# facebookresearch/vggsfm

Measured on AMD Instinct MI355X. Metric: BA LM-iterations/sec, higher is better.
Workload: dtype f64

## Files before the change

### vggsfm_amd/csrc/ba.hip

```cpp
#include <type_traits>

#include "camera_model.hpp"
#include "../../include/vggsfm_amd.h"

namespace vgg {

int cholesky_solve_enqueue(double* A, double* b, int n, double* inv_blocks, int32_t* device_fail, const int32_t* skip_flag,
                           hipStream_t st, const CholOverlap* overlap, int split_a, int split_b, const int32_t* first_blk,
                           bool flags_cleared);
int32_t* cholesky_dataflow_flags(double* ws, int n, size_t* count);
size_t cholesky_workspace_bytes(int n);
void dataflow_signal(int32_t* flag, hipStream_t st);

constexpr int kGroup = 16;
#ifndef VGG_OFFDIAG_OCC
#define VGG_OFFDIAG_OCC 3
#endif
#ifndef VGG_DIAG_OCC
#define VGG_DIAG_OCC 4
#endif
#ifndef VGG_DIAG_FULL_DEPTH
#define VGG_DIAG_FULL_DEPTH 2
#endif
#ifndef VGG_OFF_FULL_DEPTH
// ... 17 lines not shown
#ifndef VGG_CP_OCC_RHS
#define VGG_CP_OCC_RHS 2
#endif
#ifndef VGG_CP_OCC
#define VGG_CP_OCC 2
#endif
#ifndef VGG_ABLATE
#define VGG_ABLATE 0
#endif
constexpr int kSub = 32;
constexpr int kMaxWG = 2048;
constexpr int kCamSplitMax = 16;
constexpr int kCamNV = 48;
constexpr int kPackPad = 1024;

struct Ctl {
  double radius, decrease_factor, x_cost, initial_cost, gmax_cams, gmax, cand_cost, mcc, step_norm, rel;
  int32_t iteration, done, termination, need_lin, scale_ready, invalid_streak, num_succ, num_unsucc;
  int32_t linear_fail, accept, rank, world, grad_logged, pad0, pad1, pad2;
};

struct Dims {
  int C, P, O, NI, model, kd, only_k, shared, BDp, n_red, kdsh, loss;
  double loss_scale;
};

constexpr int kYc = 12;
static inline size_t y_slot_doubles(const Dims& d) { return (d.shared || d.kd == 0) ? (size_t)kYc : (size_t)d.BDp * 3; }

struct Ws {
  Ctl* ctl;
  vgg_ba_iteration* log;
  double *cand_q, *cand_t, *cand_intr, *cand_pts;
  double *scale_c, *scale_p, *colsq_c, *dsq_c, *dy;
  uint8_t* active;
  double* lin;
  double *U, *g, *costc;
  double* sys;
  double *S, *rhs;
  double* S2;
  double* gmax_pts;
  double* stepsum;
  double *G, *hs, *Ms;
  double *pdamp;
  double* T;
  double* part_B;
  double* part_F;
  double* packed;
  size_t packed_count;
  double* pk_mine;
  double* pk_gathered;
  double* cam_part;
  double* cam_split;
  double* Y;
  size_t y_bytes;
  double* chol_inv;
  double* tile_part;
  int32_t* batch_flags;
  double *Zp, *rz_part, *part_Q;
  unsigned long long* split_off;
  double* rz;
  int tile_rhs;
  double* lin_cand;
  double *U_cand, *g_cand, *cost_cand;
  size_t lin_count, sys_count, total_bytes;
};

static inline size_t align_up(size_t x, size_t a) { return (x + a - 1) / a * a; }


static Dims make_dims(const vgg_ba_problem* pb) {
  Dims d;
  d.C = pb->num_cams; d.P = pb->num_pts; d.O = pb->num_obs; d.NI = pb->num_intr; d.model = pb->camera_model;
  const int rf = pb->refine_focal ? 1 : 0, rk = (pb->refine_extra && pb->camera_model == kSimpleRadial) ? 1 : 0;
  d.kd = rf + rk;
  d.only_k = (!rf && rk) ? 1 : 0;
  d.shared = (pb->num_intr == 1) ? 1 : 0;
  d.BDp = 6 + d.kd;
  d.n_red = 6 * d.C + d.kd * d.NI;
  d.kdsh = d.shared ? d.kd : 0;
  d.loss = pb->loss; d.loss_scale = pb->loss_scale;
  return d;
}

struct Tuning { int lpp, longt, cam_wgs, point_wgs, tile_rhs; };
static Tuning g_tuning = {0, -1, 0, 0, 2};

static Ws carve(const Dims& d, int max_iters, int num_chunks, int num_segments, void* base) {
  Ws w;
  size_t off = 0;
  auto take = [&](size_t bytes) { size_t o = off; off = align_up(off + bytes, 256); return (char*)base + o; };
  w.ctl = (Ctl*)take(sizeof(Ctl));
  w.log = (vgg_ba_iteration*)take(sizeof(vgg_ba_iteration) * (size_t)(max_iters + 2));
  w.cand_q = (double*)take(8ull * 4 * d.C); w.cand_t = (double*)take(8ull * 3 * d.C);
  w.cand_intr = (double*)take(8ull * 4 * d.NI); w.cand_pts = (double*)take(8ull * 3 * d.P);
  w.scale_c = (double*)take(8ull * d.n_red); w.scale_p = (double*)take(8ull * 3 * d.P);
  w.colsq_c = (double*)take(8ull * d.n_red); w.dsq_c = (double*)take(8ull * d.n_red);
  w.dy = (double*)take(8ull * d.n_red);
  w.active = (uint8_t*)take(d.n_red);
  w.lin_count = (size_t)d.C * d.BDp * d.BDp + (size_t)d.C * d.BDp + d.C;
  w.lin = (double*)take(8ull * w.lin_count);
  w.U = w.lin; w.g = w.U + (size_t)d.C * d.BDp * d.BDp; w.costc = w.g + (size_t)d.C * d.BDp;
  w.sys_count = (size_t)d.n_red * d.n_red + d.n_red;
  w.sys = (double*)take(8ull * w.sys_count);
  w.S = w.sys; w.rhs = w.S + (size_t)d.n_red * d.n_red;
  w.S2 = (double*)take(8ull * (size_t)d.n_red * d.n_red);
  w.packed_count = (size_t)d.n_red * (d.n_red + 1) / 2 + d.n_red;
  w.packed = (double*)take(8ull * (w.packed_count + 2 * kPackPad));
  w.pk_mine = (double*)take(8ull * (w.packed_count + 2));
  w.pk_gathered = (double*)take(8ull * (w.packed_count + 3 * kPackPad));
  w.gmax_pts = (double*)take(64);
  w.stepsum = (double*)take(64);
  w.G = (double*)take(8ull * 6 * d.P); w.hs = (double*)take(8ull * 3 * d.P);
  w.pdamp = (double*)take(8ull * 3 * d.P);
  w.Ms = (double*)take(8ull * 3 * (d.kdsh ? d.kdsh : 1) * d.P);
  w.T = (double*)take(8ull * d.C * d.BDp * (1 + d.kdsh));
  w.part_B = (double*)take(8ull * kMaxWG);
  w.part_F = (double*)take(8ull * kMaxWG * 4);
  w.cam_part = (double*)take(8ull * (d.C + 1) * 3);
  w.cam_split = (double*)take(8ull * (size_t)d.C * kCamSplitMax * kCamNV);
  w.y_bytes = 8ull * ((size_t)(num_segments > 0 ? num_segments : 0) + 1) * kGroup * y_slot_doubles(d);
  w.Y = (double*)take(w.y_bytes);
  w.chol_inv = (double*)take(cholesky_workspace_bytes(d.n_red));
  {
    const size_t bdt = d.shared ? 6 : d.BDp;
    w.tile_part = (double*)take(8ull * (size_t)(num_chunks > 0 ? num_chunks : 1) * bdt * bdt * 256);
  }
  w.batch_flags = (int32_t*)take(64);
  w.Zp = (double*)take(8ull * 9 * (d.P > 0 ? d.P : 1));
  w.rz_part = (double*)take(8ull * (size_t)(num_chunks > 0 ? num_chunks : 1) * kGroup * 6 * 3);
  w.part_Q = (double*)take(8ull * kMaxWG * 8);
  w.rz = (double*)take(8ull * (size_t)((d.C + kGroup - 1) / kGroup) * kGroup * 6 * 3);
  w.split_off = (unsigned long long*)take(8ull * 2 * ((size_t)d.n_red + 2));
  w.lin_cand = (double*)take(8ull * w.lin_count);
  w.U_cand = w.lin_cand; w.g_cand = w.U_cand + (size_t)d.C * d.BDp * d.BDp; w.cost_cand = w.g_cand + (size_t)d.C * d.BDp;
  w.tile_rhs = 0;
  w.total_bytes = off;
  return w;
}

struct DevProblem {
  Dims d;
  const double *cam_q, *cam_t, *intr, *pts;
  const int32_t *row_ptr, *obs_cam, *col_ptr, *cobs_pt, *obs_slot;
  const float2 *obs_uv, *cobs_uv;
  const uint8_t *cam_const, *intr_const, *pt_const;
};

static DevProblem dev_problem(const vgg_ba_problem* pb, const Dims& d) {
  DevProblem p;
  p.d = d; p.cam_q = pb->cam_q; p.cam_t = pb->cam_t; p.intr = pb->intr; p.pts = pb->pts;
  p.row_ptr = pb->row_ptr; p.obs_cam = pb->obs_cam; p.col_ptr = pb->col_ptr; p.cobs_pt = pb->cobs_pt;
  p.obs_slot = pb->obs_slot;
  p.obs_uv = (const float2*)pb->obs_uv; p.cobs_uv = (const float2*)pb->cobs_uv;
  p.cam_const = pb->cam_const; p.intr_const = pb->intr_const; p.pt_const = pb->pt_const;
  return p;
}

template <int N>
struct ObsPf {
  static_assert(N == 2 || N == 4, "prefetch depth");
  int c0 = 0, c1 = 0, c2 = 0, c3 = 0, s0 = 0, s1 = 0, s2 = 0, s3 = 0;
  float2 u0 = make_float2(0.f, 0.f), u1 = make_float2(0.f, 0.f), u2 = make_float2(0.f, 0.f), u3 = make_float2(0.f, 0.f);
  template <bool SLOT>
  __device__ __forceinline__ void load(const int32_t* cam, const float2* uv, const int32_t* slot, int o0, int o1, int stride, int sl) {
    int o = o0 + sl;
    if (o < o1) { c0 = cam[o]; u0 = uv[o]; if (SLOT) s0 = slot[o]; }
    o += stride;
// ... 82 lines not shown
    const double s = wave_sum(v[i]);
    if (lane == 0) lds[wave * NV + i] = s;
  }
  __syncthreads();
  if (threadIdx.x < NV) out[threadIdx.x] = lds[threadIdx.x] + lds[NV + threadIdx.x] + lds[2 * NV + threadIdx.x] + lds[3 * NV + threadIdx.x];
  __syncthreads();
}

__global__ void init_kernel(DevProblem pb, Ws w, vgg_ba_options opt, int rank, int world) {
  const Dims& d = pb.d;
  const int j = blockIdx.x * blockDim.x + threadIdx.x;
  if (j == 0) {
    Ctl c;
    memset(&c, 0, sizeof(c));
    c.radius = opt.initial_trust_region_radius; c.decrease_factor = 2.0; c.need_lin = 1; c.rank = rank; c.world = world;
    *w.ctl = c;
    w.gmax_pts[0] = 0; for (int i = 0; i < 4; ++i) w.stepsum[i] = 0;
  }
  if (j < d.n_red) {
    bool act;
    if (j < 6 * d.C) {
      const int c = j / 6, k = j - 6 * c;
      const unsigned f = pb.cam_const ? pb.cam_const[c] : 0u;
      act = (pb.col_ptr[c + 1] > pb.col_ptr[c]) || world > 1;
      if (f & 1u) act = false;
      if (k >= 3 && (f & (2u << (k - 3)))) act = false;
    } else {
      const int a = (j - 6 * d.C) / d.kd;
      act = !(pb.intr_const && pb.intr_const[a]);
      if (!d.shared && world == 1 && !(pb.col_ptr[a + 1] > pb.col_ptr[a])) act = false;
    }
    w.active[j] = act ? 1 : 0;
    w.scale_c[j] = 1.0;
  }
}

__device__ __forceinline__ void zero_system_lower(const Ws& w, int n, int wg, int nwg) {
  const bool even = (n & 1) == 0;
  for (int row = wg; row <= n; row += nwg) {
    const int len = (row < n) ? min(n, 64 * (row / 64 + 1)) : n;
    double* dst = w.sys + (size_t)row * n;
    if (even) {
      double2* d2 = reinterpret_cast<double2*>(dst);
      for (int c = threadIdx.x; c < (len + 1) / 2; c += 256) d2[c] = make_double2(0.0, 0.0);
    } else {
      for (int c = threadIdx.x; c < len; c += 256) dst[c] = 0.0;
    }
  }
}

template <int KD, int MODE>
__global__ __launch_bounds__(256, (MODE == 1) ? VGG_CP_OCC_RHS : VGG_CP_OCC) void cam_pass_kernel(DevProblem pb, Ws w) {
  constexpr int BD = 6 + KD;
  constexpr int NU = BD * (BD + 1) / 2;
  constexpr int NV = (MODE == 0) ? (NU + BD + 1) : (BD * (1 + KD));
  __shared__ double red[4 * NV];
  __shared__ double tot[NV];
  if (w.ctl->done) return;
  if (MODE == 1) {
    zero_system_lower(w, pb.d.n_red, (int)(blockIdx.y * gridDim.x + blockIdx.x), (int)(gridDim.x * gridDim.y));
  }
  const Dims& d = pb.d;
  const int c = blockIdx.x, split = gridDim.y;
  double q[9], t[3], in4[4];
  quat_to_R(pb.cam_q + 4 * c, q);
#pragma unroll
// ... 188 lines not shown
  __syncthreads();
  const int n_red = pb.d.n_red;
  const double radius = ctl->radius;
#pragma unroll 4
  for (int j = threadIdx.x; j < n_red; j += 256) {
    const double sc = w.scale_c[j];
    double dd = w.colsq_c[j] * sc * sc;
    dd = fmin(fmax(dd, opt.min_lm_diagonal), opt.max_lm_diagonal);
    w.dsq_c[j] = dd / radius;
  }
}

static int lanes_per_point(int P, int O) {
  const int forced = g_tuning.lpp;
  if (forced == 8 || forced == 16 || forced == 32 || forced == 64) return forced;
  const double mean = P > 0 ? (double)O / P : 64.0;
  return mean <= 72.0 ? 16 : 32;
}
static bool long_tracks(int lpp, int P, int O) {
  return g_tuning.longt >= 0 ? g_tuning.longt != 0 : (double)O > 1.5 * lpp * (double)P;
}

template <int KD, bool LDSCAM, bool CY, int LPP, bool LONGT = false>
__global__ __launch_bounds__(256, VGG_PP_OCC) void point_pass_kernel(DevProblem pb, Ws w, vgg_ba_options opt) {
  constexpr int BD = 6 + KD;
  __shared__ double wmax[4];
  extern __shared__ double cam_cache[];
  Ctl* ctl = w.ctl;
  if (ctl->done) return;
  const Dims& d = pb.d;
  constexpr int PPW = 64 / LPP;
  const int wave = threadIdx.x >> 6, lane = threadIdx.x & 63;
  const int sub = lane / LPP, sl = lane % LPP;
  const int nw = gridDim.x * 4 * PPW;
  const bool first = !ctl->scale_ready;
  const double radius = ctl->radius;
  const int kdsh = d.kdsh;
  double gmax = 0.0;
  const bool trhs = w.tile_rhs != 0;
  if (trhs) {
    zero_system_lower(w, pb.d.n_red, (int)blockIdx.x, (int)gridDim.x);
  }
  constexpr int KQ = (KD > 0) ? KD + KD * KD : 1;
  __shared__ double qs[4][64 / LPP][KQ];
  __shared__ __attribute__((aligned(16))) double2 ystage[CY ? 4 : 1][CY ? 64 * (kYc / 2) : 1];
  __shared__ int32_t slotstage[CY ? 4 : 1][CY ? 64 : 1];
  if (trhs && KD > 0 && (lane % LPP) == 0) {
#pragma unroll
    for (int i = 0; i < KQ; ++i) qs[wave][lane / LPP][i] = 0.0;
  }
  const double* lq = cam_cache;
  const double* lt = lq + 9 * d.C;
  const double* lsc = lt + 3 * d.C;
  const double* lfl = lsc + 6 * d.C;
  if (LDSCAM) {
    for (int i = threadIdx.x; i < d.C; i += 256) {
      quat_to_R(pb.cam_q + 4 * i, cam_cache + 9 * i);
      cam_cache[18 * d.C + i] = pb.cam_const ? (double)pb.cam_const[i] : 0.0;
    }
    for (int i = threadIdx.x; i < 3 * d.C; i += 256) cam_cache[9 * d.C + i] = pb.cam_t[i];
    for (int i = threadIdx.x; i < 6 * d.C; i += 256) cam_cache[12 * d.C + i] = w.scale_c[i];
    __syncthreads();
  }
  int p = (blockIdx.x * 4 + wave) * PPW + sub;
  constexpr int NPF = LONGT ? 4 : 2;
  constexpr bool CACHEJ = !LONGT;
  int n_o0 = 0, n_o1 = 0;
  ObsPf<NPF> n_pf;
  double n_X0 = 0, n_X1 = 0, n_X2 = 0;
  int n_ptc = 0;
  int m_o0 = 0, m_o1 = 0;
  double m_X0 = 0, m_X1 = 0, m_X2 = 0;
  int m_ptc = 0;
  if (p < d.P) {
    n_o0 = pb.row_ptr[p]; n_o1 = pb.row_ptr[p + 1];
    n_X0 = pb.pts[3 * p]; n_X1 = pb.pts[3 * p + 1]; n_X2 = pb.pts[3 * p + 2];
    n_ptc = pb.pt_const ? (int)pb.pt_const[p] : 0;
    n_pf.template load<true>(pb.obs_cam, pb.obs_uv, pb.obs_slot, n_o0, n_o1, LPP, sl);
    if (p + nw < d.P) {
      const int pm = p + nw;
      m_o0 = pb.row_ptr[pm]; m_o1 = pb.row_ptr[pm + 1];
      m_X0 = pb.pts[3 * pm]; m_X1 = pb.pts[3 * pm + 1]; m_X2 = pb.pts[3 * pm + 2];
      m_ptc = pb.pt_const ? (int)pb.pt_const[pm] : 0;
    }
  }
  for (; CY ? __any(p < d.P) : (p < d.P); p += nw) {
    const bool pvalid = p < d.P;
    const int o0 = pvalid ? n_o0 : 0, o1 = pvalid ? n_o1 : 0;
    const double X[3] = {n_X0, n_X1, n_X2};
    const bool pt_c = n_ptc != 0;
    const ObsPf<NPF> f_pf = n_pf;
    {
      n_o0 = m_o0; n_o1 = m_o1; n_X0 = m_X0; n_X1 = m_X1; n_X2 = m_X2; n_ptc = m_ptc;
      if (p + nw < d.P) n_pf.template load<true>(pb.obs_cam, pb.obs_uv, pb.obs_slot, n_o0, n_o1, LPP, sl);
      const int pm = p + 2 * nw;
      if (pm < d.P) {
        m_o0 = pb.row_ptr[pm]; m_o1 = pb.row_ptr[pm + 1];
        m_X0 = pb.pts[3 * pm]; m_X1 = pb.pts[3 * pm + 1]; m_X2 = pb.pts[3 * pm + 2];
        m_ptc = pb.pt_const ? (int)pb.pt_const[pm] : 0;
      }
    }
    double V[6] = {0, 0, 0, 0, 0, 0}, g[3] = {0, 0, 0}, Wa[3 * (KD ? KD : 1)];
#pragma unroll
    for (int i = 0; i < 3 * (KD ? KD : 1); ++i) Wa[i] = 0;
    double sp[3] = {1.0, 1.0, 1.0};
    if (!first && pvalid) { sp[0] = w.scale_p[3 * (size_t)p]; sp[1] = w.scale_p[3 * (size_t)p + 1]; sp[2] = w.scale_p[3 * (size_t)p + 2]; }
    double cF[CY ? 6 : 2 * BD], cE[6];
    constexpr bool KEEPJ = CY;
    double cJ[KEEPJ ? NPF : 1][6];
    auto sweep1 = [&](const int pass, const int o, double* keepJ) __attribute__((always_inline)) {
      const bool head = pass == 0;
      const int c = f_pf.cam(pass, pb.obs_cam, o);
      const float2 uv = f_pf.uv(pass, pb.obs_uv, o);
      const int a = d.shared ? 0 : c;
      double r[2], F[2 * BD], E[6], Jw[6];
      if (LDSCAM)
        eval_full<KD>(d, lq + 9 * c, lt + 3 * c, pb.intr + 4 * a, X, uv, (unsigned)lfl[c],
                      pb.intr_const ? pb.intr_const[a] != 0 : false, pt_c, r, F, E, CY ? Jw : nullptr);
      else
        eval_full<KD>(d, CamR(pb.cam_q + 4 * c).R, pb.cam_t + 3 * c, pb.intr + 4 * a, X, uv,
                      pb.cam_const ? pb.cam_const[c] : 0u, pb.intr_const ? pb.intr_const[a] != 0 : false, pt_c, r, F, E,
                      CY ? Jw : nullptr);
      if (CACHEJ && !KEEPJ && head) {
#pragma unroll
        for (int i = 0; i < (CY ? 6 : 2 * BD); ++i) cF[i] = CY ? Jw[i] : F[i];
#pragma unroll
        for (int i = 0; i < 6; ++i) cE[i] = E[i];
      }
      if (KEEPJ && keepJ) {
// ... 924 lines not shown
          sums[KD * KD + i] += trhs ? (global_terms ? w.g[(size_t)cc * BD + 6 + i] : 0.0) : w.T[((size_t)cc * BD + 6 + i) * tw];
        }
      }
      if (trhs) {
#pragma unroll 8
        for (int b = tid; b < point_parts; b += 64) {
          const double* q = w.part_Q + 8 * (size_t)b;
#pragma unroll
          for (int i = 0; i < KD; ++i) {
#pragma unroll
            for (int j = 0; j <= i; ++j) sums[i * KD + j] -= w.scale_c[ia + i] * q[KD + i * KD + j];
            sums[KD * KD + i] -= q[i];
          }
        }
      }
#pragma unroll
      for (int i = 0; i < NS; ++i) sums[i] = wave_sum(sums[i]);
      if (tid == 0) {
#pragma unroll
        for (int i = 0; i < KD; ++i) {
#pragma unroll
          for (int j = 0; j <= i; ++j) {
            double v = sums[i * KD + j];
            if (global_terms && i == j) v += w.dsq_c[ia + i];
            w.S[(size_t)(ia + i) * n + ia + j] += v;
          }
          w.rhs[ia + i] += w.scale_c[ia + i] * sums[KD * KD + i];
        }
      }
    }
  }
}

template <int KD>
__global__ void cam_update_kernel(DevProblem pb, Ws w) {
  if (w.ctl->done) return;
  const Dims& d = pb.d;
  const int c = blockIdx.x * blockDim.x + threadIdx.x;
  if (c > d.C) return;
  double step = 0, xn = 0;
  if (c < d.C) {
    double dl[6];
    for (int k = 0; k < 6; ++k) {
      const int j = 6 * c + k;
      const double dyv = w.active[j] ? w.scale_c[j] * w.rhs[j] : 0.0;
      w.dy[j] = dyv;
      dl[k] = -dyv;
    }
    double qn[4];
    quat_plus(pb.cam_q + 4 * c, dl, qn);
    const bool pose_var = !(pb.cam_const && (pb.cam_const[c] & 1u));
    for (int k = 0; k < 4; ++k) { w.cand_q[4 * c + k] = qn[k]; const double df = qn[k] - pb.cam_q[4 * c + k]; step += df * df; if (pose_var) xn += pb.cam_q[4 * c + k] * pb.cam_q[4 * c + k]; }
    for (int k = 0; k < 3; ++k) { const double tn = pb.cam_t[3 * c + k] + dl[3 + k]; w.cand_t[3 * c + k] = tn; step += dl[3 + k] * dl[3 + k]; if (pose_var) xn += pb.cam_t[3 * c + k] * pb.cam_t[3 * c + k]; }
  }
  const int a = d.shared ? ((c == d.C) ? 0 : -1) : ((c < d.C) ? c : -1);
  if (a >= 0) {
    double in4[4];
    for (int k = 0; k < 4; ++k) in4[k] = pb.intr[4 * a + k];
    for (int k = 0; k < KD; ++k) {
      const int j = 6 * d.C + KD * a + k;
      const double dyv = w.active[j] ? w.scale_c[j] * w.rhs[j] : 0.0;
      w.dy[j] = dyv;
      const int slot = (KD == 2) ? (k == 0 ? 0 : 3) : (d.only_k ? 3 : 0);
      in4[slot] -= dyv;
      step += dyv * dyv;
    }
    const bool intr_var = KD > 0 && !(pb.intr_const && pb.intr_const[a]);
    const int np = (d.model == kSimpleRadial) ? 4 : 3;
    for (int k = 0; k < 4; ++k) { w.cand_intr[4 * a + k] = in4[k]; if (intr_var && k < np) xn += pb.intr[4 * a + k] * pb.intr[4 * a + k]; }
  }
  w.cam_part[3 * c] = step;
  w.cam_part[3 * c + 1] = xn;
  w.cam_part[3 * c + 2] = 0.0;
}

template <int KD, bool LDSCAM, int LPP, bool LONGT = false>
__global__ __launch_bounds__(256, VGG_PS_OCC) void point_step_kernel(DevProblem pb, Ws w) {
  constexpr int BD = 6 + KD;
  __shared__ double red[4][3];
  extern __shared__ double cam_cache[];
  if (w.ctl->done) return;
  const Dims& d = pb.d;
  constexpr int PPW = 64 / LPP;
  const int wave = threadIdx.x >> 6, lane = threadIdx.x & 63;
  const int sub = lane / LPP, sl = lane % LPP;
  const int nw = gridDim.x * 4 * PPW;
  double s_mcc = 0, s_step = 0, s_xn = 0;
  const double* lq = cam_cache;
  const double* lt = lq + 9 * d.C;
  const double* ldy = lt + 3 * d.C;
  const double* lfl = ldy + 6 * d.C;
  if (LDSCAM) {
    double* cc = cam_cache;
    for (int i = threadIdx.x; i < d.C; i += 256) {
      quat_to_R(pb.cam_q + 4 * i, cc + 9 * i);
      cc[18 * d.C + i] = pb.cam_const ? (double)pb.cam_const[i] : 0.0;
    }
    for (int i = threadIdx.x; i < 3 * d.C; i += 256) cc[9 * d.C + i] = pb.cam_t[i];
    for (int i = threadIdx.x; i < 6 * d.C; i += 256) cc[(ldy - cam_cache) + i] = w.dy[i];
    __syncthreads();
  }
  (void)lfl;
  int p = (blockIdx.x * 4 + wave) * PPW + sub;
  constexpr int NPF = LONGT ? 4 : 2;
  int n_o0 = 0, n_o1 = 0;
  ObsPf<NPF> n_pf;
  double n_X0 = 0, n_X1 = 0, n_X2 = 0;
  int n_ptc = 0;
  int m_o0 = 0, m_o1 = 0;
  double m_X0 = 0, m_X1 = 0, m_X2 = 0;
  int m_ptc = 0;
  if (p < d.P) {
    n_o0 = pb.row_ptr[p]; n_o1 = pb.row_ptr[p + 1];
    n_X0 = pb.pts[3 * p]; n_X1 = pb.pts[3 * p + 1]; n_X2 = pb.pts[3 * p + 2];
    n_ptc = pb.pt_const ? (int)pb.pt_const[p] : 0;
    n_pf.template load<false>(pb.obs_cam, pb.obs_uv, pb.obs_slot, n_o0, n_o1, LPP, sl);
    if (p + nw < d.P) {
      const int pm = p + nw;
      m_o0 = pb.row_ptr[pm]; m_o1 = pb.row_ptr[pm + 1];
      m_X0 = pb.pts[3 * pm]; m_X1 = pb.pts[3 * pm + 1]; m_X2 = pb.pts[3 * pm + 2];
      m_ptc = pb.pt_const ? (int)pb.pt_const[pm] : 0;
    }
  }
  for (; p < d.P; p += nw) {
    const int o0 = n_o0, o1 = n_o1;
    const double X[3] = {n_X0, n_X1, n_X2};
    const bool pt_c = n_ptc != 0;
    const ObsPf<NPF> f_pf = n_pf;
    {
      n_o0 = m_o0; n_o1 = m_o1; n_X0 = m_X0; n_X1 = m_X1; n_X2 = m_X2; n_ptc = m_ptc;
      if (p + nw < d.P) n_pf.template load<false>(pb.obs_cam, pb.obs_uv, pb.obs_slot, n_o0, n_o1, LPP, sl);
      const int pm = p + 2 * nw;
      if (pm < d.P) {
        m_o0 = pb.row_ptr[pm]; m_o1 = pb.row_ptr[pm + 1];
        m_X0 = pb.pts[3 * pm]; m_X1 = pb.pts[3 * pm + 1]; m_X2 = pb.pts[3 * pm + 2];
        m_ptc = pb.pt_const ? (int)pb.pt_const[pm] : 0;
      }
    }
    double t3[3] = {0, 0, 0};
    const double* Gp = w.G + 6 * (size_t)p;
    const double G00 = Gp[0], G01 = Gp[1], G02 = Gp[2], G11 = Gp[3], G12 = Gp[4], G22 = Gp[5];
    const double hs0 = w.hs[3 * (size_t)p], hs1 = w.hs[3 * (size_t)p + 1], hs2 = w.hs[3 * (size_t)p + 2];
    const double pd0 = w.pdamp[3 * (size_t)p], pd1 = w.pdamp[3 * (size_t)p + 1], pd2 = w.pdamp[3 * (size_t)p + 2];
    auto evaluated = [&](int pass, int o) __attribute__((always_inline)) {
      const int c = f_pf.cam(pass, pb.obs_cam, o);
      const float2 uv = f_pf.uv(pass, pb.obs_uv, o);
      const int a = d.shared ? 0 : c;
      double r[2], F[2 * BD], E[6];
      if (LDSCAM)
        eval_full<KD>(d, lq + 9 * c, lt + 3 * c, pb.intr + 4 * a, X, uv, (unsigned)lfl[c],
                      pb.intr_const ? pb.intr_const[a] != 0 : false, pt_c, r, F, E);
      else
        eval_full<KD>(d, CamR(pb.cam_q + 4 * c).R, pb.cam_t + 3 * c, pb.intr + 4 * a, X, uv,
                      pb.cam_const ? pb.cam_const[c] : 0u, pb.intr_const ? pb.intr_const[a] != 0 : false, pt_c, r, F, E);
      double fy0 = 0, fy1 = 0;
#pragma unroll
      for (int k = 0; k < 6; ++k) { const double v = LDSCAM ? ldy[6 * c + k] : w.dy[6 * c + k]; fy0 += F[k] * v; fy1 += F[BD + k] * v; }
#pragma unroll
      for (int k = 0; k < KD; ++k) { const double v = w.dy[6 * d.C + KD * a + k]; fy0 += F[6 + k] * v; fy1 += F[BD + 6 + k] * v; }
      t3[0] += E[0] * fy0 + E[3] * fy1; t3[1] += E[1] * fy0 + E[4] * fy1; t3[2] += E[2] * fy0 + E[5] * fy1;
      s_mcc += fy0 * (r[0] - 0.5 * fy0) + fy1 * (r[1] - 0.5 * fy1);
    };
    for (int o = o0 + sl; o < o1; o += LPP) evaluated((o - o0) / LPP, o);
#pragma unroll
    for (int i = 0; i < 3; ++i) t3[i] = group_sum<LPP>(t3[i]);
    const double u0 = G00 * t3[0], u1 = G01 * t3[0] + G11 * t3[1], u2 = G02 * t3[0] + G12 * t3[1] + G22 * t3[2];
    double ys[3];
    ys[0] = hs0 - (G00 * u0 + G01 * u1 + G02 * u2);
    ys[1] = hs1 - (G11 * u1 + G12 * u2);
    ys[2] = hs2 - (G22 * u2);
    if (sl == 0) {
      w.cand_pts[3 * (size_t)p] = X[0] - ys[0]; w.cand_pts[3 * (size_t)p + 1] = X[1] - ys[1]; w.cand_pts[3 * (size_t)p + 2] = X[2] - ys[2];
      s_step += ys[0] * ys[0] + ys[1] * ys[1] + ys[2] * ys[2];
      if (!pt_c) s_xn += X[0] * X[0] + X[1] * X[1] + X[2] * X[2];
      if (G22 != 0.0) {
        const double z2 = ys[2] / G22, z1 = (ys[1] - G12 * z2) / G11, z0 = (ys[0] - G01 * z1 - G02 * z2) / G00;
        s_mcc += 0.5 * (z0 * z0 + z1 * z1 + z2 * z2) + 0.5 * (pd0 * ys[0] * ys[0] + pd1 * ys[1] * ys[1] + pd2 * ys[2] * ys[2]);
      }
    }
  }
  s_mcc = wave_sum(s_mcc); s_step = wave_sum(s_step); s_xn = wave_sum(s_xn);
  if (lane == 0) { red[wave][0] = s_mcc; red[wave][1] = s_step; red[wave][2] = s_xn; }
  __syncthreads();
  if (threadIdx.x < 3) w.part_F[4 * blockIdx.x + 1 + threadIdx.x] = red[0][threadIdx.x] + red[1][threadIdx.x] + red[2][threadIdx.x] + red[3][threadIdx.x];
}

__global__ __launch_bounds__(256) void reduce_step_kernel(Ws w, int nparts, int C) {
  __shared__ double red[4][256];
  if (w.ctl->done) return;
  double s[4] = {0, 0, 0, 0};
  for (int i = threadIdx.x; i < C; i += 256) s[0] += w.cost_cand[i];
  for (int i = threadIdx.x; i < nparts; i += 256)
// ... 366 lines not shown

template <int KD>
static int phase_step(const Launch& L) {
  const Dims& d = L.d;
  size_t chol_flag_count = 0;
  int32_t* chol_flags = cholesky_dataflow_flags(L.w.chol_inv, d.n_red, &chol_flag_count);
  begin_iteration_kernel<<<1, 256, 0, L.st>>>(L.w, L.opt, d.n_red, chol_flags, (int)chol_flag_count);
  int rc;
  if (OverlapCtx* oc = overlap_ctx(L)) {
    (void)hipMemsetAsync(L.w.batch_flags, 0, 64, L.st);
    (void)hipEventRecord(oc->ready, L.st);
    (void)hipStreamWaitEvent(oc->st_rest, oc->ready, 0);
    (void)hipStreamWaitEvent(oc->st_chol, oc->ready, 0);
    launch_schur_batches<KD>(L, 1, L.num_batches, oc->st_rest, L.w.S2, L.w.batch_flags);
    CholOverlap ov;
    ov.dev_flags = L.w.batch_flags + 1;
    ov.S2 = L.w.S2;
    ov.first_col = 6 * kGroup * L.batches[6 * 1 + 5];
    ov.num_waits = L.num_batches - 1;
    for (int b = 1; b < L.num_batches; ++b) ov.wait_col[b - 1] = 6 * kGroup * L.batches[6 * b + 5];
    {
      ProfScope ps(kProfCholesky, oc->st_chol);
      rc = cholesky_solve_enqueue(L.w.S, L.w.rhs, d.n_red, L.w.chol_inv, &L.w.ctl->linear_fail, &L.w.ctl->done, oc->st_chol, &ov,
                                  L.chol_split_a, L.chol_split_b, L.chol_first_blk, true);
    }
    (void)hipEventRecord(oc->chol_done, oc->st_chol);
    (void)hipStreamWaitEvent(L.st, oc->chol_done, 0);
  } else {
    ProfScope ps(kProfCholesky, L.st);
    rc = cholesky_solve_enqueue(L.w.S, L.w.rhs, d.n_red, L.w.chol_inv, &L.w.ctl->linear_fail, &L.w.ctl->done, L.st, nullptr,
                                L.chol_split_a, L.chol_split_b, L.chol_first_blk, true);
  }
  if (rc != VGG_OK) return rc;
  cam_update_kernel<KD><<<div_up(d.C + 1, 64), 64, 0, L.st>>>(L.dp, L.w);
  {
    ProfScope ps(kProfPointStep, L.st);
    const size_t cam_lds = sizeof(double) * 19 * (size_t)d.C;
    auto launch = [&](auto lpp) {
      constexpr int LPP = decltype(lpp)::value;
      const bool longt = long_tracks(LPP, L.d.P, L.d.O);
      if (longt && LPP <= 32) {
        if (cam_lds <= 64 * 1024) point_step_kernel<KD, true, LPP, (LPP <= 32)><<<L.wgB, 256, cam_lds, L.st>>>(L.dp, L.w);
        else point_step_kernel<KD, false, LPP, (LPP <= 32)><<<L.wgB, 256, 0, L.st>>>(L.dp, L.w);
      } else if (cam_lds <= 64 * 1024) point_step_kernel<KD, true, LPP><<<L.wgB, 256, cam_lds, L.st>>>(L.dp, L.w);
      else point_step_kernel<KD, false, LPP><<<L.wgB, 256, 0, L.st>>>(L.dp, L.w);
    };
    if (L.lpp == 8) launch(std::integral_constant<int, 8>{});
    else if (L.lpp == 16) launch(std::integral_constant<int, 16>{});
    else if (L.lpp == 32) launch(std::integral_constant<int, 32>{});
    else launch(std::integral_constant<int, 64>{});
  }
  {
    ProfScope ps(kProfLinearize, L.st);
    DevProblem dc = L.dp;
    dc.cam_q = L.w.cand_q; dc.cam_t = L.w.cand_t; dc.intr = L.w.cand_intr; dc.pts = L.w.cand_pts;
    Ws wc = L.w;
    wc.U = L.w.U_cand; wc.g = L.w.g_cand; wc.costc = L.w.cost_cand;
    launch_linearize<KD>(L, dc, wc);
  }
  reduce_step_kernel<<<1, 256, 0, L.st>>>(L.w, L.wgB, d.C);
  return VGG_OK;
}

static void phase_update(const Launch& L) {
  const Dims& d = L.d;
  control_kernel<<<1, 64, 0, L.st>>>(L.w, L.opt, d.C);
  size_t nmax = (size_t)3 * d.P;
// ... 161 lines not shown
  *total_ms = tot; *launches = g_prof.n[kernel_id];
  if (reset) g_prof.n[kernel_id] = 0;
  return VGG_OK;
}

const char* vgg_build_arch(void) { return "gfx950"; }
int vgg_abi_version(void) { return VGG_ABI_VERSION; }
size_t vgg_abi_sizeof(int which) {
  switch (which) {
    case 0: return sizeof(vgg_ba_problem);
    case 1: return sizeof(vgg_ba_options);
    case 2: return sizeof(vgg_ba_iteration);
    case 3: return sizeof(vgg_ba_summary);
    default: return 0;
  }
}

size_t vgg_ba_workspace_bytes(const vgg_ba_problem* problem, const vgg_ba_options* options) {
  if (!problem || !options) return 0;
  const Dims d = make_dims(problem);
  return carve(d, options->max_num_iterations, problem->num_chunks, problem->num_segments, nullptr).total_bytes + 256;
}

int vgg_ba_begin(const vgg_ba_problem* problem, const vgg_ba_options* options, void* workspace, size_t workspace_bytes,
                 int rank, int world_size, void* stream) {
  Launch L;
  int rc = make_launch(problem, options, workspace, (hipStream_t)stream, &L);
  if (rc != VGG_OK) return rc;
  if (workspace_bytes < L.w.total_bytes) return VGG_ERR_WORKSPACE;
  if (world_size < 1 || world_size > kPackPad || rank < 0 || rank >= world_size) return VGG_ERR_INVALID_ARGUMENT;
  VGG_HIP_CHECK(hipMemsetAsync(L.w.Y, 0, L.w.y_bytes, L.st));
  VGG_HIP_CHECK(hipMemsetAsync(L.w.sys, 0, sizeof(double) * L.w.sys_count, L.st));
  init_kernel<<<div_up(L.d.n_red > 0 ? L.d.n_red : 1, 256), 256, 0, L.st>>>(L.dp, L.w, L.opt, rank, world_size);
  (void)dispatch_kd(L.d.kd, [&] { launch_linearize<0>(L, L.dp, L.w); return VGG_OK; },
                    [&] { launch_linearize<1>(L, L.dp, L.w); return VGG_OK; }, [&] { launch_linearize<2>(L, L.dp, L.w); return VGG_OK; });
  VGG_LAUNCH_CHECK();
  return VGG_OK;
}

int vgg_ba_phase(const vgg_ba_problem* problem, const vgg_ba_options* options, void* workspace, int phase, void* stream) {
  Launch L;
  int rc = make_launch(problem, options, workspace, (hipStream_t)stream, &L);
  if (rc != VGG_OK) return rc;
  rc = run_phase(L, phase);
  if (rc != VGG_OK) return rc;
  VGG_LAUNCH_CHECK();
  return VGG_OK;
}

int vgg_ba_reduce_buffer(const vgg_ba_problem* problem, const vgg_ba_options* options, void* workspace, int which,
                         double** device_ptr, size_t* count) {
  if (!problem || !options || !workspace || !device_ptr || !count) return VGG_ERR_INVALID_ARGUMENT;
  const Dims d = make_dims(problem);
  Ws w = carve(d, options->max_num_iterations, problem->num_chunks, problem->num_segments, workspace);
  switch (which) {
    case 0: *device_ptr = w.lin; *count = w.lin_count; break;
    case 1: *device_ptr = w.sys; *count = w.sys_count; break;
    case 2: *device_ptr = w.gmax_pts; *count = 1; break;
    case 3: *device_ptr = w.stepsum; *count = 4; break;
    case 4: *device_ptr = w.packed; *count = w.packed_count; break;
    case 5: *device_ptr = w.pk_mine; *count = w.packed_count + 2; break;
    case 6: *device_ptr = w.pk_gathered; *count = w.packed_count + 3 * kPackPad; break;
    case 7: *device_ptr = w.packed; *count = split_count_a(d); break;
    default: return VGG_ERR_INVALID_ARGUMENT;
  }
  return VGG_OK;
}

int vgg_ba_finish(const vgg_ba_problem* problem, const vgg_ba_options* options, void* workspace,
                  vgg_ba_summary* summary, vgg_ba_iteration* log, int log_cap, void* stream) {
  Launch L;
  int rc = make_launch(problem, options, workspace, (hipStream_t)stream, &L);
  if (rc != VGG_OK) return rc;
  return finish(L, options->max_num_iterations, summary, log, log_cap);
}

int vgg_ba_poll_done(const vgg_ba_problem* problem, const vgg_ba_options* options, void* workspace, int32_t* done_host,
                     void* stream) {
  if (!done_host) return VGG_ERR_INVALID_ARGUMENT;
  Launch L;
  int rc = make_launch(problem, options, workspace, (hipStream_t)stream, &L);
  if (rc != VGG_OK) return rc;
  int32_t done = 0;
  VGG_HIP_CHECK(hipMemcpyAsync(&done, &L.w.ctl->done, sizeof(done), hipMemcpyDeviceToHost, L.st));
  VGG_HIP_CHECK(hipStreamSynchronize(L.st));
  *done_host = done;
  return VGG_OK;
}

int vgg_ba_solve(const vgg_ba_problem* problem, const vgg_ba_options* options, void* workspace,
                 size_t workspace_bytes, vgg_ba_summary* summary, vgg_ba_iteration* log, int log_cap, void* stream) {
  int rc = vgg_ba_begin(problem, options, workspace, workspace_bytes, 0, 1, stream);
  if (rc != VGG_OK) return rc;
  Launch L;
  rc = make_launch(problem, options, workspace, (hipStream_t)stream, &L);
  if (rc != VGG_OK) return rc;
// ... 25 lines not shown
```

Measured before the change: 702.1.

## Fuse camera update into point step and balance point ranges by observation cost

Removes the separate cam_update_kernel launch and the dy buffer. A single thread per block now performs the camera and intrinsics update inside point_step_kernel, and dy is recomputed on the fly from active, scale and rhs. A new one-time prefix-sum kernel assigns each workgroup a contiguous point range balanced by observation count, replacing the grid-strided point distribution in the linearize and point-step kernels. This is meant to save a kernel launch per iteration and to even out per-block load. The cost is a serial camera update on one thread per block and a loss of the strided interleaving across blocks. The reduce-buffer query also exposes extra workspace buffers.

```diff
diff --git a/vggsfm_amd/csrc/ba.hip b/vggsfm_amd/csrc/ba.hip
--- a/vggsfm_amd/csrc/ba.hip
+++ b/vggsfm_amd/csrc/ba.hip
@@ -73,7 +73,7 @@
   Ctl* ctl;
   vgg_ba_iteration* log;
   double *cand_q, *cand_t, *cand_intr, *cand_pts;
-  double *scale_c, *scale_p, *colsq_c, *dsq_c, *dy;
+  double *scale_c, *scale_p, *colsq_c, *dsq_c;
   uint8_t* active;
   double* lin;
   double *U, *g, *costc;
@@ -104,6 +104,7 @@
   int tile_rhs;
   double* lin_cand;
   double *U_cand, *g_cand, *cost_cand;
+  int32_t* pt_first;
   size_t lin_count, sys_count, total_bytes;
 };
 
@@ -137,7 +138,6 @@
   w.cand_intr = (double*)take(8ull * 4 * d.NI); w.cand_pts = (double*)take(8ull * 3 * d.P);
   w.scale_c = (double*)take(8ull * d.n_red); w.scale_p = (double*)take(8ull * 3 * d.P);
   w.colsq_c = (double*)take(8ull * d.n_red); w.dsq_c = (double*)take(8ull * d.n_red);
-  w.dy = (double*)take(8ull * d.n_red);
   w.active = (uint8_t*)take(d.n_red);
   w.lin_count = (size_t)d.C * d.BDp * d.BDp + (size_t)d.C * d.BDp + d.C;
   w.lin = (double*)take(8ull * w.lin_count);
@@ -175,6 +175,7 @@
   w.split_off = (unsigned long long*)take(8ull * 2 * ((size_t)d.n_red + 2));
   w.lin_cand = (double*)take(8ull * w.lin_count);
   w.U_cand = w.lin_cand; w.g_cand = w.U_cand + (size_t)d.C * d.BDp * d.BDp; w.cost_cand = w.g_cand + (size_t)d.C * d.BDp;
+  w.pt_first = (int32_t*)take(4ull * (kMaxWG + 1));
   w.tile_rhs = 0;
   w.total_bytes = off;
   return w;
@@ -323,6 +324,47 @@
     }
     w.active[j] = act ? 1 : 0;
     w.scale_c[j] = 1.0;
+  }
+}
+
+constexpr unsigned kPointC0 = 5;
+__device__ __forceinline__ unsigned point_group_cost(const int32_t* row_ptr, int g, int ppw, int lpp, int P) {
+  unsigned c = 0;
+  for (int k = 0; k < ppw; ++k) {
+    const int p = g * ppw + k;
+    if (p < P) c += kPointC0 + 4u * (unsigned)((row_ptr[p + 1] - row_ptr[p] + lpp - 1) / lpp);
+  }
+  return c;
+}
+__global__ __launch_bounds__(1024) void point_ranges_kernel(DevProblem pb, Ws w, int wgB, int lpp) {
+  __shared__ unsigned long long part[1024];
+  const int P = pb.d.P, ppw = 64 / lpp, t = threadIdx.x;
+  const int NG = (P + ppw - 1) / ppw, per = (NG + 1023) / 1024;
+  const int g0 = min(t * per, NG), g1 = min(g0 + per, NG);
+  unsigned long long mine = 0;
+  for (int g = g0; g < g1; ++g) mine += point_group_cost(pb.row_ptr, g, ppw, lpp, P);
+  part[t] = mine;
+  __syncthreads();
+  for (int off = 1; off < 1024; off <<= 1) {
+    const unsigned long long v = t >= off ? part[t - off] : 0ull;
+    __syncthreads();
+    part[t] += v;
+    __syncthreads();
+  }
+  const unsigned long long total = part[1023], start = part[t] - mine, nb = (unsigned long long)wgB;
+  if (t == 0) { w.pt_first[0] = 0; w.pt_first[wgB] = P; }
+  if (NG == 0) {
+    for (int b = 1 + t; b < wgB; b += 1024) w.pt_first[b] = 0;
+    return;
+  }
+  if (g0 >= g1) return;
+  int b = g0 == 0 ? 1 : (int)(((start + 1) * nb + total - 1) / total);
+  if (b < 1) b = 1;
+  const int last = (P / ppw) * ppw;
+  unsigned long long s = start;
+  for (int g = g0; g < g1 && b < wgB; ++g) {
+    s += point_group_cost(pb.row_ptr, g, ppw, lpp, P);
+    while (b < wgB && total * (unsigned long long)b / nb <= s) { w.pt_first[b] = min((g + 1) * ppw, last); ++b; }
   }
 }
 
@@ -577,7 +619,8 @@
   constexpr int PPW = 64 / LPP;
   const int wave = threadIdx.x >> 6, lane = threadIdx.x & 63;
   const int sub = lane / LPP, sl = lane % LPP;
-  const int nw = gridDim.x * 4 * PPW;
+  constexpr int nw = 4 * PPW;
+  const int r0 = w.pt_first[blockIdx.x], r1 = w.pt_first[blockIdx.x + 1];
   const bool first = !ctl->scale_ready;
   const double radius = ctl->radius;
   const int kdsh = d.kdsh;
@@ -598,16 +641,7 @@
   const double* lt = lq + 9 * d.C;
   const double* lsc = lt + 3 * d.C;
   const double* lfl = lsc + 6 * d.C;
-  if (LDSCAM) {
-    for (int i = threadIdx.x; i < d.C; i += 256) {
-      quat_to_R(pb.cam_q + 4 * i, cam_cache + 9 * i);
-      cam_cache[18 * d.C + i] = pb.cam_const ? (double)pb.cam_const[i] : 0.0;
-    }
-    for (int i = threadIdx.x; i < 3 * d.C; i += 256) cam_cache[9 * d.C + i] = pb.cam_t[i];
-    for (int i = threadIdx.x; i < 6 * d.C; i += 256) cam_cache[12 * d.C + i] = w.scale_c[i];
-    __syncthreads();
-  }
-  int p = (blockIdx.x * 4 + wave) * PPW + sub;
+  int p = r0 + wave * PPW + sub;
   constexpr int NPF = LONGT ? 4 : 2;
   constexpr bool CACHEJ = !LONGT;
   int n_o0 = 0, n_o1 = 0;
@@ -617,29 +651,38 @@
   int m_o0 = 0, m_o1 = 0;
   double m_X0 = 0, m_X1 = 0, m_X2 = 0;
   int m_ptc = 0;
-  if (p < d.P) {
+  if (p < r1) {
     n_o0 = pb.row_ptr[p]; n_o1 = pb.row_ptr[p + 1];
     n_X0 = pb.pts[3 * p]; n_X1 = pb.pts[3 * p + 1]; n_X2 = pb.pts[3 * p + 2];
     n_ptc = pb.pt_const ? (int)pb.pt_const[p] : 0;
     n_pf.template load<true>(pb.obs_cam, pb.obs_uv, pb.obs_slot, n_o0, n_o1, LPP, sl);
-    if (p + nw < d.P) {
+    if (p + nw < r1) {
       const int pm = p + nw;
       m_o0 = pb.row_ptr[pm]; m_o1 = pb.row_ptr[pm + 1];
       m_X0 = pb.pts[3 * pm]; m_X1 = pb.pts[3 * pm + 1]; m_X2 = pb.pts[3 * pm + 2];
       m_ptc = pb.pt_const ? (int)pb.pt_const[pm] : 0;
     }
   }
-  for (; CY ? __any(p < d.P) : (p < d.P); p += nw) {
-    const bool pvalid = p < d.P;
+  if (LDSCAM) {
+    for (int i = threadIdx.x; i < d.C; i += 256) {
+      quat_to_R(pb.cam_q + 4 * i, cam_cache + 9 * i);
+      cam_cache[18 * d.C + i] = pb.cam_const ? (double)pb.cam_const[i] : 0.0;
+    }
+    for (int i = threadIdx.x; i < 3 * d.C; i += 256) cam_cache[9 * d.C + i] = pb.cam_t[i];
+    for (int i = threadIdx.x; i < 6 * d.C; i += 256) cam_cache[12 * d.C + i] = w.scale_c[i];
+    __syncthreads();
+  }
+  for (; CY ? __any(p < r1) : (p < r1); p += nw) {
+    const bool pvalid = p < r1;
     const int o0 = pvalid ? n_o0 : 0, o1 = pvalid ? n_o1 : 0;
     const double X[3] = {n_X0, n_X1, n_X2};
     const bool pt_c = n_ptc != 0;
     const ObsPf<NPF> f_pf = n_pf;
     {
       n_o0 = m_o0; n_o1 = m_o1; n_X0 = m_X0; n_X1 = m_X1; n_X2 = m_X2; n_ptc = m_ptc;
-      if (p + nw < d.P) n_pf.template load<true>(pb.obs_cam, pb.obs_uv, pb.obs_slot, n_o0, n_o1, LPP, sl);
+      if (p + nw < r1) n_pf.template load<true>(pb.obs_cam, pb.obs_uv, pb.obs_slot, n_o0, n_o1, LPP, sl);
       const int pm = p + 2 * nw;
-      if (pm < d.P) {
+      if (pm < r1) {
         m_o0 = pb.row_ptr[pm]; m_o1 = pb.row_ptr[pm + 1];
         m_X0 = pb.pts[3 * pm]; m_X1 = pb.pts[3 * pm + 1]; m_X2 = pb.pts[3 * pm + 2];
         m_ptc = pb.pt_const ? (int)pb.pt_const[pm] : 0;
@@ -1630,41 +1673,48 @@
   }
 }
 
+__device__ __forceinline__ double step_dy(const Ws& w, int j) { return w.active[j] ? w.scale_c[j] * w.rhs[j] : 0.0; }
+
 template <int KD>
-__global__ void cam_update_kernel(DevProblem pb, Ws w) {
-  if (w.ctl->done) return;
+__device__ __forceinline__ void cam_update_entry(const DevProblem& pb, const Ws& w, int c) {
   const Dims& d = pb.d;
-  const int c = blockIdx.x * blockDim.x + threadIdx.x;
-  if (c > d.C) return;
   double step = 0, xn = 0;
   if (c < d.C) {
     double dl[6];
-    for (int k = 0; k < 6; ++k) {
-      const int j = 6 * c + k;
-      const double dyv = w.active[j] ? w.scale_c[j] * w.rhs[j] : 0.0;
-      w.dy[j] = dyv;
-      dl[k] = -dyv;
-    }
-    double qn[4];
-    quat_plus(pb.cam_q + 4 * c, dl, qn);
+#pragma unroll
+    for (int k = 0; k < 6; ++k) dl[k] = -step_dy(w, 6 * c + k);
+    double q[4], qm[4], qn[4];
+#pragma unroll
+    for (int k = 0; k < 4; ++k) q[k] = pb.cam_q[4 * c + k];
+    const double nrm = sqrt(dl[0] * dl[0] + dl[1] * dl[1] + dl[2] * dl[2]);
+    const double sn = sin(nrm) / nrm;
+    const double qx = sn * dl[0], qy = sn * dl[1], qz = sn * dl[2], qw = cos(nrm);
+    qm[3] = qw * q[3] - qx * q[0] - qy * q[1] - qz * q[2];
+    qm[0] = qw * q[0] + qx * q[3] + qy * q[2] - qz * q[1];
+    qm[1] = qw * q[1] - qx * q[2] + qy * q[3] + qz * q[0];
+    qm[2] = qw * q[2] + qx * q[1] - qy * q[0] + qz * q[3];
+#pragma unroll
+    for (int k = 0; k < 4; ++k) qn[k] = nrm == 0.0 ? q[k] : qm[k];
     const bool pose_var = !(pb.cam_const && (pb.cam_const[c] & 1u));
-    for (int k = 0; k < 4; ++k) { w.cand_q[4 * c + k] = qn[k]; const double df = qn[k] - pb.cam_q[4 * c + k]; step += df * df; if (pose_var) xn += pb.cam_q[4 * c + k] * pb.cam_q[4 * c + k]; }
+#pragma unroll
+    for (int k = 0; k < 4; ++k) { w.cand_q[4 * c + k] = qn[k]; const double df = qn[k] - q[k]; step += df * df; if (pose_var) xn += q[k] * q[k]; }
+#pragma unroll
     for (int k = 0; k < 3; ++k) { const double tn = pb.cam_t[3 * c + k] + dl[3 + k]; w.cand_t[3 * c + k] = tn; step += dl[3 + k] * dl[3 + k]; if (pose_var) xn += pb.cam_t[3 * c + k] * pb.cam_t[3 * c + k]; }
   }
   const int a = d.shared ? ((c == d.C) ? 0 : -1) : ((c < d.C) ? c : -1);
   if (a >= 0) {
     double in4[4];
+#pragma unroll
     for (int k = 0; k < 4; ++k) in4[k] = pb.intr[4 * a + k];
+#pragma unroll
     for (int k = 0; k < KD; ++k) {
-      const int j = 6 * d.C + KD * a + k;
-      const double dyv = w.active[j] ? w.scale_c[j] * w.rhs[j] : 0.0;
-      w.dy[j] = dyv;
-      const int slot = (KD == 2) ? (k == 0 ? 0 : 3) : (d.only_k ? 3 : 0);
-      in4[slot] -= dyv;
+      const double dyv = step_dy(w, 6 * d.C + KD * a + k);
+      if ((KD == 2) ? (k == 0) : !d.only_k) in4[0] -= dyv; else in4[3] -= dyv;
       step += dyv * dyv;
     }
     const bool intr_var = KD > 0 && !(pb.intr_const && pb.intr_const[a]);
     const int np = (d.model == kSimpleRadial) ? 4 : 3;
+#pragma unroll
     for (int k = 0; k < 4; ++k) { w.cand_intr[4 * a + k] = in4[k]; if (intr_var && k < np) xn += pb.intr[4 * a + k] * pb.intr[4 * a + k]; }
   }
   w.cam_part[3 * c] = step;
@@ -1676,30 +1726,22 @@
 __global__ __launch_bounds__(256, VGG_PS_OCC) void point_step_kernel(DevProblem pb, Ws w) {
   constexpr int BD = 6 + KD;
   __shared__ double red[4][3];
+  __shared__ double dyi[KD > 0 ? KD : 1];
   extern __shared__ double cam_cache[];
   if (w.ctl->done) return;
   const Dims& d = pb.d;
   constexpr int PPW = 64 / LPP;
   const int wave = threadIdx.x >> 6, lane = threadIdx.x & 63;
   const int sub = lane / LPP, sl = lane % LPP;
-  const int nw = gridDim.x * 4 * PPW;
+  constexpr int nw = 4 * PPW;
+  const int r0 = w.pt_first[blockIdx.x], r1 = w.pt_first[blockIdx.x + 1];
   double s_mcc = 0, s_step = 0, s_xn = 0;
   const double* lq = cam_cache;
   const double* lt = lq + 9 * d.C;
   const double* ldy = lt + 3 * d.C;
   const double* lfl = ldy + 6 * d.C;
-  if (LDSCAM) {
-    double* cc = cam_cache;
-    for (int i = threadIdx.x; i < d.C; i += 256) {
-      quat_to_R(pb.cam_q + 4 * i, cc + 9 * i);
-      cc[18 * d.C + i] = pb.cam_const ? (double)pb.cam_const[i] : 0.0;
-    }
-    for (int i = threadIdx.x; i < 3 * d.C; i += 256) cc[9 * d.C + i] = pb.cam_t[i];
-    for (int i = threadIdx.x; i < 6 * d.C; i += 256) cc[(ldy - cam_cache) + i] = w.dy[i];
-    __syncthreads();
-  }
   (void)lfl;
-  int p = (blockIdx.x * 4 + wave) * PPW + sub;
+  int p = r0 + wave * PPW + sub;
   constexpr int NPF = LONGT ? 4 : 2;
   int n_o0 = 0, n_o1 = 0;
   ObsPf<NPF> n_pf;
@@ -1708,28 +1750,42 @@
   int m_o0 = 0, m_o1 = 0;
   double m_X0 = 0, m_X1 = 0, m_X2 = 0;
   int m_ptc = 0;
-  if (p < d.P) {
+  if (p < r1) {
     n_o0 = pb.row_ptr[p]; n_o1 = pb.row_ptr[p + 1];
     n_X0 = pb.pts[3 * p]; n_X1 = pb.pts[3 * p + 1]; n_X2 = pb.pts[3 * p + 2];
     n_ptc = pb.pt_const ? (int)pb.pt_const[p] : 0;
     n_pf.template load<false>(pb.obs_cam, pb.obs_uv, pb.obs_slot, n_o0, n_o1, LPP, sl);
-    if (p + nw < d.P) {
+    if (p + nw < r1) {
       const int pm = p + nw;
       m_o0 = pb.row_ptr[pm]; m_o1 = pb.row_ptr[pm + 1];
       m_X0 = pb.pts[3 * pm]; m_X1 = pb.pts[3 * pm + 1]; m_X2 = pb.pts[3 * pm + 2];
       m_ptc = pb.pt_const ? (int)pb.pt_const[pm] : 0;
     }
   }
-  for (; p < d.P; p += nw) {
+  if (threadIdx.x == 255) {
+    for (int c = blockIdx.x; c <= d.C; c += gridDim.x) cam_update_entry<KD>(pb, w, c);
+  }
+  if (LDSCAM) {
+    double* cc = cam_cache;
+    for (int i = threadIdx.x; i < d.C; i += 256) {
+      quat_to_R(pb.cam_q + 4 * i, cc + 9 * i);
+      cc[18 * d.C + i] = pb.cam_const ? (double)pb.cam_const[i] : 0.0;
+    }
+    for (int i = threadIdx.x; i < 3 * d.C; i += 256) cc[9 * d.C + i] = pb.cam_t[i];
+    for (int i = threadIdx.x; i < 6 * d.C; i += 256) cc[(ldy - cam_cache) + i] = step_dy(w, i);
+  }
+  if (KD > 0 && d.shared && threadIdx.x < KD) dyi[threadIdx.x] = step_dy(w, 6 * d.C + threadIdx.x);
+  __syncthreads();
+  for (; p < r1; p += nw) {
     const int o0 = n_o0, o1 = n_o1;
     const double X[3] = {n_X0, n_X1, n_X2};
     const bool pt_c = n_ptc != 0;
     const ObsPf<NPF> f_pf = n_pf;
     {
       n_o0 = m_o0; n_o1 = m_o1; n_X0 = m_X0; n_X1 = m_X1; n_X2 = m_X2; n_ptc = m_ptc;
-      if (p + nw < d.P) n_pf.template load<false>(pb.obs_cam, pb.obs_uv, pb.obs_slot, n_o0, n_o1, LPP, sl);
+      if (p + nw < r1) n_pf.template load<false>(pb.obs_cam, pb.obs_uv, pb.obs_slot, n_o0, n_o1, LPP, sl);
       const int pm = p + 2 * nw;
-      if (pm < d.P) {
+      if (pm < r1) {
         m_o0 = pb.row_ptr[pm]; m_o1 = pb.row_ptr[pm + 1];
         m_X0 = pb.pts[3 * pm]; m_X1 = pb.pts[3 * pm + 1]; m_X2 = pb.pts[3 * pm + 2];
         m_ptc = pb.pt_const ? (int)pb.pt_const[pm] : 0;
@@ -1753,9 +1809,9 @@
                       pb.cam_const ? pb.cam_const[c] : 0u, pb.intr_const ? pb.intr_const[a] != 0 : false, pt_c, r, F, E);
       double fy0 = 0, fy1 = 0;
 #pragma unroll
-      for (int k = 0; k < 6; ++k) { const double v = LDSCAM ? ldy[6 * c + k] : w.dy[6 * c + k]; fy0 += F[k] * v; fy1 += F[BD + k] * v; }
-#pragma unroll
-      for (int k = 0; k < KD; ++k) { const double v = w.dy[6 * d.C + KD * a + k]; fy0 += F[6 + k] * v; fy1 += F[BD + 6 + k] * v; }
+      for (int k = 0; k < 6; ++k) { const double v = LDSCAM ? ldy[6 * c + k] : step_dy(w, 6 * c + k); fy0 += F[k] * v; fy1 += F[BD + k] * v; }
+#pragma unroll
+      for (int k = 0; k < KD; ++k) { const double v = d.shared ? dyi[k] : step_dy(w, 6 * d.C + KD * a + k); fy0 += F[6 + k] * v; fy1 += F[BD + 6 + k] * v; }
       t3[0] += E[0] * fy0 + E[3] * fy1; t3[1] += E[1] * fy0 + E[4] * fy1; t3[2] += E[2] * fy0 + E[5] * fy1;
       s_mcc += fy0 * (r[0] - 0.5 * fy0) + fy1 * (r[1] - 0.5 * fy1);
     };
@@ -2188,7 +2244,6 @@
                                 L.chol_split_a, L.chol_split_b, L.chol_first_blk, true);
   }
   if (rc != VGG_OK) return rc;
-  cam_update_kernel<KD><<<div_up(d.C + 1, 64), 64, 0, L.st>>>(L.dp, L.w);
   {
     ProfScope ps(kProfPointStep, L.st);
     const size_t cam_lds = sizeof(double) * 19 * (size_t)d.C;
@@ -2416,6 +2471,7 @@
   VGG_HIP_CHECK(hipMemsetAsync(L.w.Y, 0, L.w.y_bytes, L.st));
   VGG_HIP_CHECK(hipMemsetAsync(L.w.sys, 0, sizeof(double) * L.w.sys_count, L.st));
   init_kernel<<<div_up(L.d.n_red > 0 ? L.d.n_red : 1, 256), 256, 0, L.st>>>(L.dp, L.w, L.opt, rank, world_size);
+  point_ranges_kernel<<<1, 1024, 0, L.st>>>(L.dp, L.w, L.wgB, L.lpp);
   (void)dispatch_kd(L.d.kd, [&] { launch_linearize<0>(L, L.dp, L.w); return VGG_OK; },
                     [&] { launch_linearize<1>(L, L.dp, L.w); return VGG_OK; }, [&] { launch_linearize<2>(L, L.dp, L.w); return VGG_OK; });
   VGG_LAUNCH_CHECK();
@@ -2446,6 +2502,13 @@
     case 5: *device_ptr = w.pk_mine; *count = w.packed_count + 2; break;
     case 6: *device_ptr = w.pk_gathered; *count = w.packed_count + 3 * kPackPad; break;
     case 7: *device_ptr = w.packed; *count = split_count_a(d); break;
+    case 8: *device_ptr = (double*)w.pt_first; *count = kMaxWG + 1; break;
+    case 9: *device_ptr = w.cand_q; *count = 4 * (size_t)d.C; break;
+    case 10: *device_ptr = w.cand_t; *count = 3 * (size_t)d.C; break;
+    case 11: *device_ptr = w.cand_intr; *count = 4 * (size_t)d.NI; break;
+    case 12: *device_ptr = w.cam_part; *count = 3 * ((size_t)d.C + 1); break;
+    case 13: *device_ptr = w.scale_c; *count = (size_t)d.n_red; break;
+    case 14: *device_ptr = (double*)w.active; *count = (size_t)d.n_red; break;
     default: return VGG_ERR_INVALID_ARGUMENT;
   }
   return VGG_OK;
```

Result: no change. 697.1 (-0.7%).
